# bitsauce/Carla-ppo

Hardware: AMD Instinct MI355X
Metric: VAE+PPO train frames/sec on 160×80×3 synthetic obs at 1/2/4/8 MI355X (higher is better)
Workload: dtype bf16; 1 GPU; ConvVAE SGD step (fwd+ELBO+bwd+TF-Adam), batch=512 per GPU, 160x80x3 frames, z_dim=64, rgb target (BASELINE configs[1]; global batch 512); global_batch=512, parallelism=single, frames_resident_in_hbm=2048, frame_table=uint8 camera bytes, k/255 in registers, noise=N(0,1) drawn inside the reparameterisation kernel (Philox4x32-10), launch=eager launches: one C call per step (mi_vae_train_step), storage=bf16 activations/weights, fp32 accumulate, fp32 master weights+Adam

## Files before the change

carla-ppo_amd/csrc/conv_ops.hip:

```cpp
#include <stdlib.h>
#include "gemm_core.hpp"
#include "tallk_tile.hpp"
#include "mi_internal.hpp"
#include "mi355_carla.h"

using namespace mi;

namespace {

inline int esz_of(int dtype) { return dtype == MI_BF16 ? 2 : 4; }
inline bool dtype_ok(int dtype) { return dtype == MI_F32 || dtype == MI_BF16 || dtype == MI_BF16X3; }

template <typename T, typename TIn, int AMODE, int BMODE, int VA, int AALIGN>
int launch_gemm_bn(hipStream_t st, const GemmParams& p, int M_for_grid, int gz) {
    const int gx = (M_for_grid + GEMM_BM - 1) / GEMM_BM;
    if (gx <= 0) return MI_OK;
    if (p.N <= 32) {
        dim3 g(gx, 1, gz);
        MI_LAUNCH((gemm_kernel<T, TIn, AMODE, BMODE, VA, AALIGN, 32>), g, dim3(GEMM_NT), 0, st, p);
    } else if (p.N <= 64) {
        dim3 g(gx, 1, gz);
        MI_LAUNCH((gemm_kernel<T, TIn, AMODE, BMODE, VA, AALIGN, 64>), g, dim3(GEMM_NT), 0, st, p);
    } else {
        dim3 g(gx, (p.N + 127) / 128, gz);
// ... 711 lines not shown
    if (nslab < 1 || n < 1) return MI_OK;
    const MiSlabSum job = {slabs, out, stride, n, nslab, overwrite};
    if (!list || st != list->stream) return sr_launch(st, &job, 1);
    if (list->njobs == MI_SMALL_SUMS_MAX) { const int rc = mi_small_sums_flush(list); if (rc != MI_OK) return rc; }
    list->job[list->njobs++] = job;
    return MI_OK;
}
int mi_tiled_reduces_flush(MiTiledReduces* l, MiSmallSums* small) {
    TiledStore& t = tiled_store(l);
    const int n = l->nreduce, nf = l->nfold;
    l->nreduce = 0; l->nfold = 0;
    int rc = MI_OK;
    if (n == 1 || n > TW_MAX_FUSED) {
        for (int i = 0; i < n; ++i) launch_tiled_reduce(l->stream, t.reduce[i], small);
        rc = mi_check_launch("reduce_tiled_kernel");
    } else if (n > 0) {
        FusedReduceParams& f = t.fused;
        f.n = n; f.first[0] = 0; f.bias.njobs = 0; f.bias.first[0] = 0; f.bias.ovw = 0;
        for (int i = 0; i < n; ++i) {
            const PendingReduce& r = t.reduce[i];
            f.q[i] = r.q; f.splits[i] = r.splits; f.ngroups[i] = r.ngroups; f.kind[i] = r.kind; f.ry[i] = (int)reduce_ry(r);
            f.first[i + 1] = f.first[i] + (int)reduce_blocks(r, (unsigned)f.ry[i]);
            if (r.bpart && f.bias.njobs < SR_MAX) sr_add(f.bias, r.bpart, (long long)r.bN, r.bnslab, (long long)r.bN, r.bout);
        }
        for (int i = n; i < TW_MAX_FUSED; ++i) f.first[i + 1] = f.first[n];
        for (int i = f.bias.njobs; i < SR_MAX; ++i) f.bias.first[i + 1] = f.bias.first[f.bias.njobs];
        MI_LAUNCH(reduce_fused_kernel, dim3((unsigned)(f.first[n] + f.bias.first[f.bias.njobs])), dim3(256), 0, l->stream, f);
        rc = mi_check_launch("reduce_fused_kernel");
    }
    if (nf > 0 && rc == MI_OK && small && small->stream == l->stream) rc = mi_small_sums_flush(small);
    for (int i = 0; i < nf && rc == MI_OK; ++i) rc = launch_fold(l->stream, t.fold[i]);
    return rc;
}

void mi_get_trace(long long** buf, int* cap) { *buf = g_trace; *cap = g_trace_cap; }

extern "C" {

int mi_debug_set_trace(void* dev_ptr, int capacity_entries) { g_trace = (long long*)dev_ptr; g_trace_cap = dev_ptr ? capacity_entries : 0; return MI_OK; }

int mi_debug_wgrad_unreduced(void* stream, int deconv, int dtype, const void* t0, int B, int H, int W, int C0, const void* t1, int K, int C1, float* dw, void* scratch, long long scratch_bytes, float* dbias) {
    MiTiledReduces dropped(stream);
    const MiWgradCtx cx = {&dropped, nullptr, 0, 0};
    return deconv ? mi_deconv2d_nhwc_wgrad_ctx(stream, dtype, t0, B, H, W, C0, t1, K, K, C1, dw, scratch, scratch_bytes, dbias, &cx)
                  : mi_conv2d_nhwc_wgrad_ctx(stream, dtype, t0, nullptr, 0, B, H, W, C0, t1, K, K, C1, dw, scratch, scratch_bytes, dbias, &cx);
}

int mi_conv2d_nhwc_fwd(void* stream, int dtype, const void* x, const int* frame_idx, int x_is_f32,
                       int B, int IH, int IW, int Cin, const void* w, int w_transposed, const float* bias, int KH, int KW, int Cout,
                       int relu, void* out) {
    return mi_conv2d_nhwc_fwd_bits(stream, dtype, x, frame_idx, x_is_f32, B, IH, IW, Cin, w, w_transposed, bias, KH, KW, Cout, relu, out, nullptr, nullptr);
}

int mi_conv2d_nhwc_fwd_bits(void* stream, int dtype, const void* x, const int* frame_idx, int x_is_f32,
                            int B, int IH, int IW, int Cin, const void* w, int w_transposed, const float* bias, int KH, int KW, int Cout,
                            int relu, void* out, void* relu_bits, int* wrote_bits) {
    const void* const wfrag = mi_rwconv_take_wfrag();
    const int OH = (IH - KH) / 2 + 1, OW = (IW - KW) / 2 + 1;
    if (wrote_bits) *wrote_bits = 0;
    if (w_transposed) {
        const int r4 = try_narrow_conv((hipStream_t)stream, dtype, x, x_is_f32 == 2 ? 2 : ((x_is_f32 || dtype == MI_F32) ? 1 : (dtype == MI_BF16X3 ? 3 : 0)), frame_idx, w, B, IH, IW, Cin, KH, KW, Cout, bias, relu, nullptr, out,
                                       (dtype == MI_BF16 && relu && Cout == 32) ? relu_bits : nullptr);
        if (r4 > 0 && wrote_bits && relu_bits && dtype == MI_BF16 && relu && Cout == 32) *wrote_bits = 1;
        if (r4 != 0) return r4 > 0 ? MI_OK : r4;
    }
    if (x_is_f32 == 2) return mi_fail(MI_ERR_ARG, "mi_conv2d_nhwc_fwd: uint8 frames are only read by the narrow-layer kernel (bf16 mode, 1..3 channels -> 32, K-contiguous weights)");
    GemmParams p = {};
    p.a = x; p.a_frame_idx = frame_idx;
    fill_conv_geom(p, B, IH, IW, Cin, OH, OW, KH, KW, 2, needs_merge(Cin, dtype, x_is_f32));
    p.N = Cout; p.b = w; p.ldb = w_transposed ? p.K : Cout; p.b_vec = vec_ok(w, p.ldb, dtype);
    p.out = out; p.bias = bias; p.mask = nullptr; p.relu = relu; p.out_f32 = 0; p.ksplit_len = 0;
    if (w_transposed) return conv_form_gemm<B_NK>((hipStream_t)stream, dtype, x_is_f32, p, 1, wfrag);
    return conv_form_gemm<B_KN>((hipStream_t)stream, dtype, x_is_f32, p, 1);
}

int mi_conv2d_nhwc_dgrad(void* stream, int dtype, const void* dy, int B, int OH, int OW, int Cout,
                         const void* w, int KH, int KW, int Cin, int IH, int IW, const void* mask, void* dx) {
    return mi_conv2d_nhwc_dgrad_bits(stream, dtype, dy, B, OH, OW, Cout, w, KH, KW, Cin, IH, IW, mask, nullptr, dx);
}

int mi_conv2d_nhwc_dgrad_bits(void* stream, int dtype, const void* dy, int B, int OH, int OW, int Cout,
                              const void* w, int KH, int KW, int Cin, int IH, int IW, const void* mask, const void* mask_bits, void* dx) {
    if (mask_bits) {
        const int r5 = mi_try_rwconv_gather((hipStream_t)stream, dtype, dy, w, B, OH, OW, Cout, IH, IW, Cin, KH, KW, dx, nullptr, mask, 0, mask_bits, nullptr, nullptr);
        if (r5 != 0) return r5 > 0 ? MI_OK : r5;
    }
    GemmParams p = {};
    p.a = dy; p.b = w; p.ldb = 0; p.b_vec = 1;
    p.out = dx; p.bias = nullptr; p.mask = mask; p.relu = 0; p.out_f32 = 0;
    return deconv_form_gemm((hipStream_t)stream, dtype, p, B, OH, OW, Cout, IH, IW, Cin, KH, KW);
}

int mi_conv2d_nhwc_wgrad(void* stream, int dtype, const void* x, const int* frame_idx, int x_is_f32,
                         int B, int IH, int IW, int Cin, const void* dy, int KH, int KW, int Cout, float* dw) {
    return mi_conv2d_nhwc_wgrad_ctx(stream, dtype, x, frame_idx, x_is_f32, B, IH, IW, Cin, dy, KH, KW, Cout, dw, nullptr, 0, nullptr, nullptr);
}

int mi_conv2d_nhwc_wgrad_ws(void* stream, int dtype, const void* x, const int* frame_idx, int x_is_f32,
                            int B, int IH, int IW, int Cin, const void* dy, int KH, int KW, int Cout, float* dw, void* scratch, long long scratch_bytes,
                            float* dbias) {
    return mi_conv2d_nhwc_wgrad_ctx(stream, dtype, x, frame_idx, x_is_f32, B, IH, IW, Cin, dy, KH, KW, Cout, dw, scratch, scratch_bytes, dbias, nullptr);
}
int mi_conv2d_nhwc_wgrad_ctx(void* stream, int dtype, const void* x, const int* frame_idx, int x_is_f32, int B, int IH, int IW, int Cin, const void* dy, int KH, int KW, int Cout,
                             float* dw, void* scratch, long long scratch_bytes, float* dbias, const MiWgradCtx* ctx) {
    const int OH = (IH - KH) / 2 + 1, OW = (IW - KW) / 2 + 1;
    {
        const int r4 = try_narrow_wgrad((hipStream_t)stream, dtype, x, x_is_f32 == 2 ? 2 : ((x_is_f32 || dtype == MI_F32) ? 1 : 0), frame_idx, dy, B, IH, IW, Cin, OH, OW, Cout, KH, KW, dw, dbias, scratch, scratch_bytes, ctx);
        if (r4 != 0) return r4 > 0 ? MI_OK : r4;
    }
    if (x_is_f32 == 2) return mi_fail(MI_ERR_ARG, "mi_conv2d_nhwc_wgrad: uint8 frames are only read by the narrow-layer kernel (bf16 mode)");
    if (!frame_idx && !x_is_f32) {
        const int r3 = dtype == MI_BF16X3 ? try_tapwgrad_split((hipStream_t)stream, TC_CONV, x, dy, B, IH, IW, Cin, OH, OW, Cout, KH, KW, dw, scratch, scratch_bytes, dbias, ctx)
                                          : try_tapwgrad((hipStream_t)stream, dtype, TC_CONV, x, dy, B, IH, IW, Cin, OH, OW, Cout, KH, KW, dw, scratch, scratch_bytes, dbias, ctx);
        if (r3 != 0) return r3 > 0 ? MI_OK : r3;
    }
    if (dbias) {
        long long cb = (mi_colsum_scratch_bytes(dtype, (long long)B * OH * OW, Cout) + 255) / 256 * 256;
        if (!scratch || cb > scratch_bytes) cb = 0;
        const int rcb = mi_colsum_ctx(stream, dtype, dy, (long long)B * OH * OW, Cout, dbias, cb ? scratch : nullptr, cb, ctx);
        if (rcb != MI_OK) return rcb;
        if (cb) { scratch = (char*)scratch + cb; scratch_bytes -= cb; }
    }
    WgradParams p = {};
    p.big = x; p.frame_idx = frame_idx;
    fill_wgrad_geom(p, B, IH, IW, Cin, OH, OW, KH, KW, 2, needs_merge(Cin, dtype, x_is_f32));
    p.N = Cout; p.small = dy; p.s_vec = vec_ok(dy, Cout, dtype); p.out = dw;
    return launch_wgrad((hipStream_t)stream, dtype, x_is_f32, p, 1024, scratch, scratch_bytes, 0, ctx);
}

int mi_deconv2d_nhwc_fwd(void* stream, int dtype, const void* x, int B, int IH, int IW, int Cin,
                         const void* w, const float* bias, int KH, int KW, int Cout, int relu, void* out) {
    return mi_deconv2d_nhwc_fwd_bits(stream, dtype, x, B, IH, IW, Cin, w, bias, KH, KW, Cout, relu, out, nullptr, nullptr);
}

int mi_deconv2d_nhwc_fwd_bits(void* stream, int dtype, const void* x, int B, int IH, int IW, int Cin,
                              const void* w, const float* bias, int KH, int KW, int Cout, int relu, void* out, void* relu_bits, int* wrote_bits) {
    const void* const wfrag = mi_rwconv_take_wfrag();
    if (wrote_bits) *wrote_bits = 0;
    if (relu_bits && relu) {
        const int r5 = mi_try_rwconv_gather((hipStream_t)stream, dtype, x, w, B, IH, IW, Cin, (IH - 1) * 2 + KH, (IW - 1) * 2 + KW, Cout, KH, KW, out, bias, nullptr, relu, nullptr, relu_bits, wfrag);
        if (r5 > 0 && wrote_bits) *wrote_bits = 1;
        if (r5 != 0) return r5 > 0 ? MI_OK : r5;
    }
    const int OH = (IH - 1) * 2 + KH, OW = (IW - 1) * 2 + KW;
    GemmParams p = {};
    p.a = x; p.b = w; p.ldb = 0; p.b_vec = 1;
    p.out = out; p.bias = bias; p.mask = nullptr; p.relu = relu; p.out_f32 = 0;
    return deconv_form_gemm((hipStream_t)stream, dtype, p, B, IH, IW, Cin, OH, OW, Cout, KH, KW, wfrag);
}

int mi_deconv2d_nhwc_fwd_bce(void* stream, int dtype, const void* x, int B, int IH, int IW, int Cin, const void* w, const float* bias, int KH, int KW, int Cout,
                             void* logits, const float* labels, const int* frame_idx, long long label_stride, int loss_kind, float inv_batch, void* dlogits,
                             float* loss_partial, float* bias_partial, int partial_capacity, int* n_partial) {
    return mi_deconv2d_nhwc_fwd_bce_u8(stream, dtype, x, B, IH, IW, Cin, w, bias, KH, KW, Cout, logits, labels, 0, frame_idx, label_stride, loss_kind, inv_batch, dlogits,
                                       loss_partial, bias_partial, partial_capacity, n_partial);
}

int mi_deconv2d_nhwc_fwd_bce_u8(void* stream, int dtype, const void* x, int B, int IH, int IW, int Cin, const void* w, const float* bias, int KH, int KW, int Cout,
                                void* logits, const void* labels_any, int labels_u8, const int* frame_idx, long long label_stride, int loss_kind, float inv_batch, void* dlogits,
                                float* loss_partial, float* bias_partial, int partial_capacity, int* n_partial) {
    const float* labels = (const float*)labels_any;
    if (!n_partial || !labels || !loss_partial || !bias_partial) return mi_fail(MI_ERR_ARG, "mi_deconv2d_nhwc_fwd_bce: missing buffers");
    *n_partial = 0;
    if (loss_kind < 0 || loss_kind > 2) return mi_fail(MI_ERR_ARG, "mi_deconv2d_nhwc_fwd_bce: loss_kind must be 0 (bce), 1 (bce_v2) or 2 (mse)");
    const int OH = (IH - 1) * 2 + KH, OW = (IW - 1) * 2 + KW;
    NarrowLoss L = {labels, frame_idx, label_stride, loss_kind, inv_batch, dlogits, loss_partial, bias_partial, partial_capacity, 0, labels_u8 ? 1 : 0};
    const int r = try_gather_narrow((hipStream_t)stream, dtype, x, w, B, IH, IW, Cin, OH, OW, Cout, KH, KW, logits, bias, nullptr, 0, &L);
    if (r < 0) return r;
    if (r > 0) *n_partial = L.nblocks;
    return MI_OK;
}

static int dectail_grid(int fast) {
    static int resident[2];
    if (!resident[fast]) {
        int per_cu = 0, dev = 0, cus = 256;
        hipDeviceProp_t pr;
        const void* fn = fast ? (const void*)dectail_kernel<true> : (const void*)dectail_kernel<false>;
        if (hipOccupancyMaxActiveBlocksPerMultiprocessor(&per_cu, fn, 256, 0) != hipSuccess || per_cu < 1) per_cu = 2;
        if (hipGetDevice(&dev) == hipSuccess && hipGetDeviceProperties(&pr, dev) == hipSuccess) cus = pr.multiProcessorCount;
        resident[fast] = per_cu * cus;
    }
    return resident[fast];
}
int mi_deconv2d_tail_blocks(void) { const int a = dectail_grid(0), b = dectail_grid(1); return a > b ? a : b; }

int mi_deconv2d_tail_fused(void* stream, int dtype, const void* x, int B, int IH, int IW, int Cin, const void* w, const void* w_t, const float* bias, int KH, int KW, int Cout,
                           const void* labels, int labels_u8, const int* frame_idx, long long label_stride, int loss_kind, float inv_batch,
                           void* dx, float* dw, float* loss_partial, float* bias_partial, int partial_capacity, int* n_partial, void* scratch, long long scratch_bytes, int reduce_now) {
    if (!n_partial || !labels || !loss_partial || !bias_partial || !x || !w || !w_t || !dx || !dw) return mi_fail(MI_ERR_ARG, "mi_deconv2d_tail_fused: missing buffers");
    *n_partial = 0;
    if (loss_kind < 0 || loss_kind > 2) return mi_fail(MI_ERR_ARG, "mi_deconv2d_tail_fused: loss_kind must be 0 (bce), 1 (bce_v2) or 2 (mse)");
    if (!knob(K_DECTAIL) || !knob(K_NARROW) || dtype != MI_BF16 || Cin != 32 || Cout != 3 || KH != 4 || KW != 4 || B < 1 || IH < 1 || IW < 1) return MI_OK;
    if (((((uintptr_t)x) | ((uintptr_t)w) | ((uintptr_t)w_t) | ((uintptr_t)dx) | ((uintptr_t)scratch) | ((uintptr_t)dw)) & 15) || !scratch) return MI_OK;
    if ((3 * (2 * IW + 2)) % 4 != 0 || label_stride % 4 != 0 || (((uintptr_t)labels) & (labels_u8 ? 3 : 15))) return MI_OK;
    DecTailParams q = {};
    q.x = (const bf16_t*)x; q.B = B; q.IH = IH; q.IW = IW; q.w = (const bf16_t*)w; q.wt = (const bf16_t*)w_t; q.bias = bias;
    q.labels = labels; q.lab_u8 = labels_u8 ? 1 : 0; q.lab_idx = frame_idx; q.lab_stride = label_stride; q.loss_kind = loss_kind; q.inv_b = inv_batch;
    q.dx = (bf16_t*)dx; q.lpart = loss_partial; q.bpart = bias_partial;
    q.OH = 2 * IH + 2; q.OW = 2 * IW + 2; q.GH = IH + 1; q.GW = IW + 1;
    const int edge = knob(K_DECTAIL_EDGE);
    q.edge_own = edge;
    if ((long long)B * IH * IW * 64 >= 0x7fffff00ll || (long long)q.OH * q.OW * 12 >= 0x7fffff00ll) return MI_OK;
    q.x_bytes = (unsigned)((long long)B * IH * IW * 64);
    const int tiles_y = ((edge ? IH : q.GH) + DT_TY - 1) / DT_TY;
    q.tiles_x = ((edge ? IW : q.GW) + DT_TX - 1) / DT_TX; q.tiles_per_frame = tiles_y * q.tiles_x;
    const long long ntiles = (long long)B * q.tiles_per_frame;
    if (ntiles >= (1ll << 30) || (long long)B * q.OH * q.OW * 3 >= (1ll << 40)) return MI_OK;
    q.ntiles = (int)ntiles; q.div_tpf = make_fastdiv(q.tiles_per_frame); q.div_tx = make_fastdiv(q.tiles_x);
    const int fast = loss_kind == 0 ? 1 : 0;
    int nblocks = dectail_grid(fast);
    if (nblocks > q.ntiles) nblocks = q.ntiles;
    if (nblocks >= 16) nblocks &= ~7;
    if (nblocks > partial_capacity || scratch_bytes < (long long)nblocks * DT_SLAB * 4) return MI_OK;
    q.slabs = (float*)scratch;
    q.dbg = knob(K_DECTAIL_DBG);
    if (fast && q.dbg) MI_LAUNCH((dectail_kernel<true, true>), dim3(nblocks), dim3(256), 0, (hipStream_t)stream, q);
    else if (fast && knob(K_DECTAIL_SPLIT5)) MI_LAUNCH((dectail_kernel<true, false, true>), dim3(nblocks), dim3(256), 0, (hipStream_t)stream, q);
    else if (fast) MI_LAUNCH(dectail_kernel<true>, dim3(nblocks), dim3(256), 0, (hipStream_t)stream, q);
    else MI_LAUNCH(dectail_kernel<false>, dim3(nblocks), dim3(256), 0, (hipStream_t)stream, q);
    int rc = mi_check_launch("dectail_kernel");
    if (rc != MI_OK) return rc;
    if (reduce_now) rc = mi_deconv2d_tail_reduce_ctx(stream, scratch, nblocks, dw, nullptr);
    if (rc == MI_OK) *n_partial = nblocks;
    return rc;
}

int mi_deconv2d_tail_reduce(void* stream, const void* scratch, int n_partial, float* dw) { return mi_deconv2d_tail_reduce_ctx(stream, scratch, n_partial, dw, nullptr); }
int mi_deconv2d_tail_reduce_ctx(void* stream, const void* scratch, int n_partial, float* dw, const MiWgradCtx* ctx) {
    if (!scratch || !dw || n_partial < 1) return mi_fail(MI_ERR_ARG, "mi_deconv2d_tail_reduce: missing buffers");
    if (small_of(ctx)) return mi_reduce_slabs((hipStream_t)stream, (const float*)scratch, (long long)DT_SLAB, n_partial, (long long)DT_SLAB, dw, 0, ctx->small);
    MI_LAUNCH(dectail_reduce_kernel, dim3(DT_SLAB / 32), dim3(1024), 0, (hipStream_t)stream, (const float*)scratch, n_partial, dw);
    return mi_check_launch("dectail_reduce_kernel");
}

int mi_deconv2d_nhwc_dgrad(void* stream, int dtype, const void* dy, int B, int OH, int OW, int Cout,
                           const void* w, int w_transposed, int KH, int KW, int Cin, const void* mask, void* dx) {
    return mi_deconv2d_nhwc_dgrad_bits(stream, dtype, dy, B, OH, OW, Cout, w, w_transposed, KH, KW, Cin, mask, nullptr, dx);
}

int mi_deconv2d_nhwc_dgrad_bits(void* stream, int dtype, const void* dy, int B, int OH, int OW, int Cout,
                                const void* w, int w_transposed, int KH, int KW, int Cin, const void* mask, const void* mask_bits, void* dx) {
    const void* const wfrag = mi_rwconv_take_wfrag();
    const int IH = (OH - KH) / 2 + 1, IW = (OW - KW) / 2 + 1;
    if (w_transposed) {
        const int r4 = try_narrow_conv((hipStream_t)stream, dtype, dy, dtype == MI_F32 ? 1 : (dtype == MI_BF16X3 ? 3 : 0), nullptr, w, B, OH, OW, Cout, KH, KW, Cin, nullptr, 0, mask, dx, nullptr, mask_bits);
        if (r4 != 0) return r4 > 0 ? MI_OK : r4;
    }
    GemmParams p = {};
    p.a = dy; p.a_frame_idx = nullptr;
    fill_conv_geom(p, B, OH, OW, Cout, IH, IW, KH, KW, 2, needs_merge(Cout, dtype, 0));
    p.N = Cin; p.b = w; p.ldb = w_transposed ? p.K : Cin; p.b_vec = vec_ok(w, p.ldb, dtype);
    p.out = dx; p.bias = nullptr; p.mask = mask; p.relu = 0; p.out_f32 = 0; p.ksplit_len = 0;
    if (w_transposed) return conv_form_gemm<B_NK>((hipStream_t)stream, dtype, 0, p, 1, wfrag);
    return conv_form_gemm<B_KN>((hipStream_t)stream, dtype, 0, p, 1);
}

int mi_deconv2d_nhwc_wgrad(void* stream, int dtype, const void* dy, int B, int OH, int OW, int Cout,
                           const void* x, int KH, int KW, int Cin, float* dw) {
    return mi_deconv2d_nhwc_wgrad_ctx(stream, dtype, dy, B, OH, OW, Cout, x, KH, KW, Cin, dw, nullptr, 0, nullptr, nullptr);
}

int mi_deconv2d_nhwc_wgrad_ws(void* stream, int dtype, const void* dy, int B, int OH, int OW, int Cout,
                              const void* x, int KH, int KW, int Cin, float* dw, void* scratch, long long scratch_bytes, float* dbias) {
    return mi_deconv2d_nhwc_wgrad_ctx(stream, dtype, dy, B, OH, OW, Cout, x, KH, KW, Cin, dw, scratch, scratch_bytes, dbias, nullptr);
}
int mi_deconv2d_nhwc_wgrad_ctx(void* stream, int dtype, const void* dy, int B, int OH, int OW, int Cout, const void* x, int KH, int KW, int Cin,
                               float* dw, void* scratch, long long scratch_bytes, float* dbias, const MiWgradCtx* ctx) {
    const int IH = (OH - KH) / 2 + 1, IW = (OW - KW) / 2 + 1;
    {
        const int r4 = dbias ? 0 : try_narrow_wgrad((hipStream_t)stream, dtype, dy, 0, nullptr, x, B, OH, OW, Cout, IH, IW, Cin, KH, KW, dw, nullptr, scratch, scratch_bytes, ctx);
        if (r4 != 0) return r4 > 0 ? MI_OK : r4;
    }
    {
        const int r3 = dtype == MI_BF16X3 ? try_tapwgrad_split((hipStream_t)stream, TC_GATHER, x, dy, B, IH, IW, Cin, OH, OW, Cout, KH, KW, dw, scratch, scratch_bytes, dbias, ctx)
                                          : try_tapwgrad((hipStream_t)stream, dtype, TC_GATHER, x, dy, B, IH, IW, Cin, OH, OW, Cout, KH, KW, dw, scratch, scratch_bytes, dbias, ctx);
        if (r3 != 0) return r3 > 0 ? MI_OK : r3;
    }
    if (dbias) {
        long long cb = (mi_colsum_scratch_bytes(dtype, (long long)B * OH * OW, Cout) + 255) / 256 * 256;
        if (!scratch || cb > scratch_bytes) cb = 0;
        const int rcb = mi_colsum_ctx(stream, dtype, dy, (long long)B * OH * OW, Cout, dbias, cb ? scratch : nullptr, cb, ctx);
        if (rcb != MI_OK) return rcb;
        if (cb) { scratch = (char*)scratch + cb; scratch_bytes -= cb; }
    }
    WgradParams p = {};
    p.big = dy; p.frame_idx = nullptr;
    fill_wgrad_geom(p, B, OH, OW, Cout, IH, IW, KH, KW, 2, needs_merge(Cout, dtype, 0));
    p.N = Cin; p.small = x; p.s_vec = vec_ok(x, Cin, dtype); p.out = dw;
    return launch_wgrad((hipStream_t)stream, dtype, 0, p, 1024, scratch, scratch_bytes, 0, ctx);
}

int mi_gemm_bias_act(void* stream, int dtype, const void* a, int M, int K, const void* w, int w_layout, int N,
                     const float* bias, int relu, const void* mask, void* out, int out_f32, int nsplit) {
    if (dtype == MI_F32 && w_layout == 0 && nsplit <= 1 && !mask && M <= 256 && K % 4 == 0 && knob(K_GEMM2) &&
        ((((uintptr_t)a) | ((uintptr_t)out)) & 15) == 0) {
        DenseSmallParams q = {(const float*)a, (const float*)w, bias, (float*)out, M, N, K, relu};
        MI_LAUNCH(dense_smallm_kernel, dim3((N + 31) / 32, (M + 31) / 32), dim3(256), 0, (hipStream_t)stream, q);
        return mi_check_launch("dense_smallm_kernel");
    }
    if (dtype == MI_BF16 && w_layout == 1 && nsplit > 1 && out_f32 && !bias && !relu && !mask && knob(K_TALLK) && (N == 32 || N == 64 || N == 128) &&
        K % (nsplit * 16) == 0 && ((((uintptr_t)a) | ((uintptr_t)w)) & 15) == 0 && (long long)M * K * 2 < (1ll << 30) && (long long)N * K * 2 < (1ll << 30)) {
        const int nt = N / 32, kp = 4 / nt;
        if (nsplit % kp == 0) {
            TallKParams q = {a, w, (float*)out, M, N, K, K / nsplit, (unsigned)((long long)M * K * 2), (unsigned)((long long)N * K * 2)};
            const dim3 g((M + 31) / 32, nsplit / kp);
            if (nt == 4) MI_LAUNCH(tallk_kernel<4>, g, dim3(256), 0, (hipStream_t)stream, q);
            else if (nt == 2) MI_LAUNCH(tallk_kernel<2>, g, dim3(256), 0, (hipStream_t)stream, q);
            else MI_LAUNCH(tallk_kernel<1>, g, dim3(256), 0, (hipStream_t)stream, q);
            return mi_check_launch("tallk_kernel");
        }
    }
    GemmParams p = {};
    p.a = a; p.a_frame_idx = nullptr;
    fill_conv_geom(p, M, 1, 1, K, 1, 1, 1, 1, 1, false);
    const int vb = dtype == MI_BF16 ? 8 : 4;
    if (K % vb != 0) return mi_fail(MI_ERR_SHAPE, "mi_gemm_bias_act: K must be a multiple of the 16-byte vector (pad K)");
    p.N = N; p.b = w; p.ldb = w_layout == 0 ? N : K; p.b_vec = vec_ok(w, p.ldb, dtype);
    p.out = out; p.bias = bias; p.mask = mask; p.relu = relu; p.out_f32 = out_f32;
    int gz = 1;
    if (nsplit > 1) {
        if (bias || relu || mask || !out_f32) return mi_fail(MI_ERR_ARG, "mi_gemm_bias_act: split-K writes raw fp32 slabs only");
        const int bk = dtype == MI_BF16 ? 32 : 16;
        int len = (K + nsplit - 1) / nsplit;
        len = ((len + bk - 1) / bk) * bk;
        if ((long long)len * (nsplit - 1) >= K) return mi_fail(MI_ERR_ARG, "mi_gemm_bias_act: nsplit too large for K (empty slab)");
        p.ksplit_len = len; gz = nsplit;
    }
    if (w_layout == 0) return conv_form_gemm<B_KN>((hipStream_t)stream, dtype, 0, p, gz);
    return conv_form_gemm<B_NK>((hipStream_t)stream, dtype, 0, p, gz);
}

int mi_gemm_wgrad(void* stream, int dtype, const void* a, const void* dy, int M, int K, int N, float* dw) {
    return mi_gemm_wgrad_ws(stream, dtype, a, dy, M, K, N, dw, nullptr, 0);
}

static bool dwgs_eligible(int dtype, int M, int K, int N) {
    return knob(K_DWGS) && dtype == MI_BF16 && M >= 16 && M % 16 == 0 && K % 64 == 0 && N % 64 == 0 && (long long)K * N <= 262144 &&
           (long long)M * K < (1ll << 31) && (long long)M * N < (1ll << 31);
}
static int dwgs_wsplit(int M) {
    const int steps = M / 16;
    if (steps % 4 == 0 && steps / 4 >= 2) return 4;
    if (steps % 2 == 0 && steps / 2 >= 2) return 2;
    return 1;
}

long long mi_gemm_wgrad_scratch_bytes(int dtype, int M, int K, int N) {
    if (M < 1 || K < 1 || N < 1) return 0;
    const int splits = wgrad_splits(dtype, M, K + 1, N, knob(K_DENSE_WGRAD_BLOCKS), nullptr);
    return splits > 1 ? (long long)splits * (((long long)(K + 1) * N + 3) / 4 * 4) * 4 : 0;
}

int mi_gemm_wgrad_ws(void* stream, int dtype, const void* a, const void* dy, int M, int K, int N, float* dw, void* scratch, long long scratch_bytes) {
    return mi_gemm_wgrad_bias_ws(stream, dtype, a, dy, M, K, N, dw, nullptr, scratch, scratch_bytes);
}

int mi_gemm_wgrad_bias_ws(void* stream, int dtype, const void* a, const void* dy, int M, int K, int N, float* dw, float* dbias, void* scratch, long long scratch_bytes) {
    return mi_gemm_wgrad_bias_ctx(stream, dtype, a, dy, M, K, N, dw, dbias, scratch, scratch_bytes, 0, nullptr);
}

int mi_gemm_wgrad_bias_set(void* stream, int dtype, const void* a, const void* dy, int M, int K, int N, float* dw, float* dbias, void* scratch, long long scratch_bytes, int overwrite) {
    return mi_gemm_wgrad_bias_ctx(stream, dtype, a, dy, M, K, N, dw, dbias, scratch, scratch_bytes, overwrite, nullptr);
}
int mi_gemm_wgrad_bias_ctx(void* stream, int dtype, const void* a, const void* dy, int M, int K, int N, float* dw, float* dbias, void* scratch, long long scratch_bytes, int overwrite, const MiWgradCtx* ctx) {
    if (overwrite && knob(K_DWG) && dtype == MI_BF16 && M >= 1 && K % 128 == 0 && N % 128 == 0 && (long long)(K / 128) * (N / 128) >= 256 &&
        ((((uintptr_t)a) | ((uintptr_t)dy) | ((uintptr_t)dw)) & 15) == 0 && fits_desc((long long)M * K * 2) && fits_desc((long long)M * N * 2)) {
        DwgParams q = {a, (uint32_t)((long long)M * K * 2), dy, (uint32_t)((long long)M * N * 2), dw, dbias, M, K, N, K / 128, N / 128};
        const int per = (q.KT * q.NT + 7) / 8;
        if (knob(K_DWG_NST) == 3) MI_LAUNCH(dwg_kernel<3>, dim3((unsigned)(per * 8)), dim3(256), 0, (hipStream_t)stream, q);
        else MI_LAUNCH(dwg_kernel<4>, dim3((unsigned)(per * 8)), dim3(256), 0, (hipStream_t)stream, q);
        return mi_check_launch("dwg_kernel");
    }
    if (dwgs_eligible(dtype, M, K, N)) {
        DwgsParams q = {(const bf16_t*)a, (const bf16_t*)dy, dw, dbias, M, K, N, K / 64, N / 64, overwrite ? 1 : 0};
        const int per = (q.KT * q.NT + 7) / 8, ws = dwgs_wsplit(M);
        if (overwrite) MI_LAUNCH(dwgs_kernel<true>, dim3((unsigned)(per * 8)), dim3(64 * ws), 0, (hipStream_t)stream, q);
        else MI_LAUNCH(dwgs_kernel<false>, dim3((unsigned)(per * 8)), dim3(64 * ws), 0, (hipStream_t)stream, q);
        return mi_check_launch("dwgs_kernel");
    }
    WgradParams p = {};
    p.ones_row = dbias ? 1 : 0; p.dbias = dbias;
    p.big = a; p.frame_idx = nullptr;
    fill_wgrad_geom(p, M, 1, 1, K, 1, 1, 1, 1, 1, false);
    const int vb = dtype == MI_BF16 ? 8 : 4;
    if (K % vb != 0) return mi_fail(MI_ERR_SHAPE, "mi_gemm_wgrad: K must be a multiple of the 16-byte vector (pad K)");
    p.N = N; p.small = dy; p.s_vec = vec_ok(dy, N, dtype); p.out = dw;
    return launch_wgrad((hipStream_t)stream, dtype, 0, p, knob(K_DENSE_WGRAD_BLOCKS), scratch, scratch_bytes, overwrite, ctx);
}

int mi_gemm_wgrad_bias_pair_ws(void* stream, int dtype, const void* a0, const void* dy0, int M0, int K0, int N0, float* dw0, float* db0, void* scratch0, long long scratch_bytes0,
                               const void* a1, const void* dy1, int M1, int K1, int N1, float* dw1, float* db1, void* scratch1, long long scratch_bytes1) {
    return mi_gemm_wgrad_bias_pair_ctx(stream, dtype, a0, dy0, M0, K0, N0, dw0, db0, scratch0, scratch_bytes0, a1, dy1, M1, K1, N1, dw1, db1, scratch1, scratch_bytes1, nullptr);
}
int mi_gemm_wgrad_bias_pair_ctx(void* stream, int dtype, const void* a0, const void* dy0, int M0, int K0, int N0, float* dw0, float* db0, void* scratch0, long long scratch_bytes0,
                                const void* a1, const void* dy1, int M1, int K1, int N1, float* dw1, float* db1, void* scratch1, long long scratch_bytes1, const MiWgradCtx* ctx) {
    const void* A[2] = {a0, a1}; const void* DY[2] = {dy0, dy1}; const int M[2] = {M0, M1}, K[2] = {K0, K1}, N[2] = {N0, N1};
    float* DW[2] = {dw0, dw1}; float* DB[2] = {db0, db1}; void* WS[2] = {scratch0, scratch1}; const long long NB[2] = {scratch_bytes0, scratch_bytes1};
    bool ok = dtype == MI_BF16;
    WgradPair q = {};
    dim3 g[2];
    for (int i = 0; i < 2 && ok; ++i) {
        if (dwgs_eligible(dtype, M[i], K[i], N[i]) || K[i] % 8 != 0 || (((uintptr_t)A[i]) & 15)) { ok = false; break; }
        WgradParams& p = q.p[i];
        p.ones_row = DB[i] ? 1 : 0; p.dbias = DB[i];
        p.big = A[i]; p.frame_idx = nullptr;
        fill_wgrad_geom(p, M[i], 1, 1, K[i], 1, 1, 1, 1, 1, false);
        p.N = N[i]; p.small = DY[i]; p.s_vec = vec_ok(DY[i], N[i], dtype); p.out = DW[i];
        bool wide = false;
        if (prepare_wgrad(dtype, p, knob(K_DENSE_WGRAD_BLOCKS), WS[i], NB[i], 0, &g[i], &wide) != MI_OK || !wide || p.C % 8 != 0) ok = false;
    }
    if (!ok) {
        const int rc = mi_gemm_wgrad_bias_ctx(stream, dtype, a0, dy0, M0, K0, N0, dw0, db0, scratch0, scratch_bytes0, 0, ctx);
        return rc != MI_OK ? rc : mi_gemm_wgrad_bias_ctx(stream, dtype, a1, dy1, M1, K1, N1, dw1, db1, scratch1, scratch_bytes1, 0, ctx);
    }
    q.n0 = (int)(g[0].x * g[0].y * g[0].z);
    for (int i = 0; i < 2; ++i) { q.gx[i] = (int)g[i].x; q.gy[i] = (int)g[i].y; }
    const unsigned nblk = (unsigned)q.n0 + g[1].x * g[1].y * g[1].z;
    MI_LAUNCH((wgrad_pair_kernel<bf16_t, bf16_t, 8, 16, 128>), dim3(nblk), dim3(GEMM_NT), 0, (hipStream_t)stream, q);
    int rc = mi_check_launch("wgrad_pair_kernel");
    for (int i = 0; i < 2 && rc == MI_OK; ++i) {
        const WgradParams& p = q.p[i];
        if (!p.slabs) continue;
        rc = mi_reduce_slabs((hipStream_t)stream, p.slabs, p.slab_stride, (int)g[i].z, (long long)p.Kc * p.N, p.out, 0, small_of(ctx));
        if (rc == MI_OK && p.ones_row) rc = mi_reduce_slabs((hipStream_t)stream, p.slabs + (long long)p.Kc * p.N, p.slab_stride, (int)g[i].z, (long long)p.N, p.dbias, 0, small_of(ctx));
    }
    return rc;
}

}
```

carla-ppo_amd/csrc/tallk_tile.hpp:

```cpp
#pragma once
#include "common.hpp"

namespace mi {

struct TallKParams {
    const void* a; const void* wt; float* out;
    int M, N, K, len;
    unsigned a_bytes, w_bytes;
};

template <int NT>
__global__ __launch_bounds__(256) void tallk_kernel(const TallKParams p) {
    constexpr int KP = 4 / NT;
    const int lane = threadIdx.x & 63, wave = threadIdx.x >> 6, lrow = lane & 31, lgrp = lane >> 5;
    const int nt = wave % NT, kp = wave / NT;
    const int m0 = blockIdx.x * 32, slab = blockIdx.y * KP + kp;
    const int k0 = slab * p.len;
    const __amdgpu_buffer_rsrc_t rsA = __builtin_amdgcn_make_buffer_rsrc((void*)p.a, 0, (int)p.a_bytes, 0x00020000);
    const __amdgpu_buffer_rsrc_t rsW = __builtin_amdgcn_make_buffer_rsrc((void*)p.wt, 0, (int)p.w_bytes, 0x00020000);
    const unsigned arow = (unsigned)min(m0 + lrow, p.M - 1) * (unsigned)p.K, wrow = (unsigned)(nt * 32 + lrow) * (unsigned)p.K;
    f32x16 acc;
#pragma unroll
    for (int r = 0; r < 16; ++r) acc[r] = 0.f;
    constexpr int U = 6;
    const int steps = p.len >> 4;
    for (int s0 = 0; s0 < steps; s0 += U) {
        u16x8 fa[U], fb[U];
#pragma unroll
        for (int u = 0; u < U; ++u) {
            const unsigned k = (unsigned)(k0 + (s0 + u) * 16 + lgrp * 8);
            const bool on = s0 + u < steps;
            fa[u] = __builtin_bit_cast(u16x8, __builtin_amdgcn_raw_buffer_load_b128(rsA, on ? (int)((arow + k) * 2u) : (int)0x40000000, 0, 0));
            fb[u] = __builtin_bit_cast(u16x8, __builtin_amdgcn_raw_buffer_load_b128(rsW, on ? (int)((wrow + k) * 2u) : (int)0x40000000, 0, 0));
        }
#pragma unroll
        for (int u = 0; u < U; ++u) acc = __builtin_amdgcn_mfma_f32_32x32x16_bf16(__builtin_bit_cast(bf16x8, fa[u]), __builtin_bit_cast(bf16x8, fb[u]), acc, 0, 0, 0);
    }
    float* const o = p.out + ((long long)slab * p.M) * p.N + nt * 32 + lrow;
#pragma unroll
    for (int r = 0; r < 16; ++r) {
        const int m = m0 + (r & 3) + 8 * (r >> 2) + 4 * lgrp;
        if (m < p.M) o[(long long)m * p.N] = acc[r];
    }
}

}
```

Baseline: 637,900 frames/s.

## Add round-based tall-K GEMM kernel with deeper load batches and per-slab blocks

Adds a tall-K split-GEMM kernel that issues a whole round of buffer loads (24 steps for N=128, 6 for narrower N) ahead of a sched_barrier, then runs the MFMAs. The aim is more memory-level parallelism per wave. Each block now covers exactly one K slab with NT waves, so the grid grows for N=32/64 instead of packing several K slabs into one 256-thread block. The 24-deep load round raises VGPR pressure and may reduce occupancy.

```diff
diff --git a/carla-ppo_amd/csrc/conv_ops.hip b/carla-ppo_amd/csrc/conv_ops.hip
--- a/carla-ppo_amd/csrc/conv_ops.hip
+++ b/carla-ppo_amd/csrc/conv_ops.hip
@@ -1037,8 +1037,15 @@
     if (dtype == MI_BF16 && w_layout == 1 && nsplit > 1 && out_f32 && !bias && !relu && !mask && knob(K_TALLK) && (N == 32 || N == 64 || N == 128) &&
         K % (nsplit * 16) == 0 && ((((uintptr_t)a) | ((uintptr_t)w)) & 15) == 0 && (long long)M * K * 2 < (1ll << 30) && (long long)N * K * 2 < (1ll << 30)) {
         const int nt = N / 32, kp = 4 / nt;
+        TallKParams q = {a, w, (float*)out, M, N, K, K / nsplit, (unsigned)((long long)M * K * 2), (unsigned)((long long)N * K * 2)};
+        if (TALLK_ROUNDS) {
+            const dim3 g((M + 31) / 32, nsplit);
+            if (nt == 4) MI_LAUNCH((tallk_round_kernel<4, TALLK_ROUND>), g, dim3(256), 0, (hipStream_t)stream, q);
+            else if (nt == 2) MI_LAUNCH((tallk_round_kernel<2, TALLK_ROUND_SHARED>), g, dim3(128), 0, (hipStream_t)stream, q);
+            else MI_LAUNCH((tallk_round_kernel<1, TALLK_ROUND_SHARED>), g, dim3(64), 0, (hipStream_t)stream, q);
+            return mi_check_launch("tallk_round_kernel");
+        }
         if (nsplit % kp == 0) {
-            TallKParams q = {a, w, (float*)out, M, N, K, K / nsplit, (unsigned)((long long)M * K * 2), (unsigned)((long long)N * K * 2)};
             const dim3 g((M + 31) / 32, nsplit / kp);
             if (nt == 4) MI_LAUNCH(tallk_kernel<4>, g, dim3(256), 0, (hipStream_t)stream, q);
             else if (nt == 2) MI_LAUNCH(tallk_kernel<2>, g, dim3(256), 0, (hipStream_t)stream, q);
diff --git a/carla-ppo_amd/csrc/tallk_tile.hpp b/carla-ppo_amd/csrc/tallk_tile.hpp
--- a/carla-ppo_amd/csrc/tallk_tile.hpp
+++ b/carla-ppo_amd/csrc/tallk_tile.hpp
@@ -44,4 +44,50 @@
     }
 }
 
+constexpr bool TALLK_ROUNDS = true;
+constexpr int TALLK_ROUND = 24;
+constexpr int TALLK_ROUND_SHARED = 6;
+
+template <int R, bool FULL>
+__device__ __forceinline__ void tallk_round(const __amdgpu_buffer_rsrc_t rsA, const __amdgpu_buffer_rsrc_t rsW, const unsigned va, const unsigned vw, const int left, f32x16& acc) {
+    constexpr int G = 6;
+    static_assert(R % G == 0, "a round is whole groups");
+    u16x8 fa[R], fb[R];
+#pragma unroll
+    for (int u = 0; u < R; ++u) {
+        const bool on = FULL || u < left;
+        fa[u] = __builtin_bit_cast(u16x8, __builtin_amdgcn_raw_buffer_load_b128(rsA, (int)((on ? va : 0x40000000u) + (unsigned)u * 32u), 0, 0));
+        fb[u] = __builtin_bit_cast(u16x8, __builtin_amdgcn_raw_buffer_load_b128(rsW, (int)((on ? vw : 0x40000000u) + (unsigned)u * 32u), 0, 0));
+    }
+    __builtin_amdgcn_sched_barrier(0);
+#pragma unroll
+    for (int g = 0; g < R; g += G) {
+        if (!FULL && g >= left) break;
+#pragma unroll
+        for (int u = g; u < g + G; ++u) acc = __builtin_amdgcn_mfma_f32_32x32x16_bf16(__builtin_bit_cast(bf16x8, fa[u]), __builtin_bit_cast(bf16x8, fb[u]), acc, 0, 0, 0);
+    }
 }
+
+template <int NT, int R>
+__global__ __launch_bounds__(NT * 64) void tallk_round_kernel(const TallKParams p) {
+    const int lane = threadIdx.x & 63, nt = threadIdx.x >> 6, lrow = lane & 31, lgrp = lane >> 5;
+    const int row0 = blockIdx.x * 32, slab = blockIdx.y;
+    const __amdgpu_buffer_rsrc_t rsA = __builtin_amdgcn_make_buffer_rsrc((void*)p.a, 0, (int)p.a_bytes, 0x00020000);
+    const __amdgpu_buffer_rsrc_t rsW = __builtin_amdgcn_make_buffer_rsrc((void*)p.wt, 0, (int)p.w_bytes, 0x00020000);
+    const unsigned k = (unsigned)(slab * p.len + lgrp * 8);
+    unsigned va = ((unsigned)min(row0 + lrow, p.M - 1) * (unsigned)p.K + k) * 2u, vw = ((unsigned)(nt * 32 + lrow) * (unsigned)p.K + k) * 2u;
+    f32x16 acc;
+#pragma unroll
+    for (int r = 0; r < 16; ++r) acc[r] = 0.f;
+    int left = p.len >> 4;
+    for (; left >= R; left -= R, va += R * 32, vw += R * 32) tallk_round<R, true>(rsA, rsW, va, vw, left, acc);
+    if (left > 0) tallk_round<R, false>(rsA, rsW, va, vw, left, acc);
+    float* const o = p.out + ((long long)slab * p.M) * p.N + nt * 32 + lrow;
+#pragma unroll
+    for (int r = 0; r < 16; ++r) {
+        const int m = row0 + (r & 3) + 8 * (r >> 2) + 4 * lgrp;
+        if (m < p.M) o[(long long)m * p.N] = acc[r];
+    }
+}
+
+}
```

Result: no change. 639,200 frames/s (median of 5 runs) (+0.2%).
